# alexj94/future_urban_scene_generation

Hardware: AMD Instinct MI355X
Metric: synthesised vehicle crops/sec @256x256 (higher is better)
Workload: dtype f32 tensors; conv contraction as 3 fp16 MFMA products of scaled (hi, lo) operand splits, f32 accumulate (error vs fp64 <= 1.3x the exact-f32 MFMA kernel's: observed 0.96-1.27x over 12 operand scales x 5 layers; range-guarded; exact-f32 leg in precision_legs)

## Files before the change

### future_urban_scene_generation_amd/_lib.py

```python
from __future__ import annotations

import ctypes as C
import os

_HERE = os.path.dirname(os.path.abspath(__file__))
LIB_PATH = os.environ.get("FUSG_LIB", os.path.join(_HERE, "libfusg.so"))


class FusgUnavailable(RuntimeError):
    pass


class FusgError(RuntimeError):
    pass


class Tensor(C.Structure):
    _fields_ = [("data", C.c_void_p),
                ("n", C.c_int64), ("c", C.c_int64), ("h", C.c_int64), ("w", C.c_int64),
                ("sn", C.c_int64), ("sc", C.c_int64), ("sh", C.c_int64), ("sw", C.c_int64),
                ("dtype", C.c_int32), ("_pad", C.c_int32)]


class ConvDesc(C.Structure):
# ... 72 lines not shown
    "fusg_set_route_batch": (C.c_int, [C.c_int32]),
    "fusg_route_batch": (C.c_int32, []),
    "fusg_conv2d_route_order": (C.c_int, [C.POINTER(ConvDesc), C.POINTER(C.c_int32 * 4)]),
    "fusg_hg_bottleneck": (C.c_int, [C.POINTER(BneckDesc), C.c_void_p]),
    "fusg_vunet_respair": (C.c_int, [C.POINTER(RespairDesc), C.c_void_p]),
    "fusg_hg_head": (C.c_int, [C.POINTER(HgHeadDesc), C.c_void_p]),
    "fusg_conv2d_entry_nin": (C.c_int, [C.POINTER(ConvDesc), C.POINTER(ConvDesc), C.c_void_p]),
    "fusg_conv2d_entry_nin_route": (C.c_int, [C.POINTER(ConvDesc), C.POINTER(ConvDesc)]),
    "fusg_chan_stats": (C.c_int, [_TP, C.c_void_p, C.c_int32, C.c_void_p]),
    "fusg_in_finalize": (C.c_int, [_TP, C.c_void_p, C.c_int32, C.c_float, C.c_void_p, C.c_void_p, C.c_void_p]),
    "fusg_ln_finalize": (C.c_int, [_TP, C.c_void_p, C.c_int32, C.c_float, C.c_void_p, C.c_void_p, C.c_void_p,
                                   C.c_void_p, C.c_void_p]),
    "fusg_in_finalize_slots": (C.c_int, [C.c_void_p, C.c_int32, C.c_int32, C.c_int32, C.c_float, C.c_void_p, C.c_void_p, C.c_void_p]),
    "fusg_ln_finalize_slots": (C.c_int, [C.c_void_p, C.c_int32, C.c_int32, C.c_int32, C.c_float, C.c_void_p, C.c_void_p,
                                         C.c_void_p, C.c_void_p, C.c_void_p]),
    "fusg_affine_act": (C.c_int, [_TP, C.c_void_p, C.c_void_p, C.c_int64, C.c_int32, _TP, _TP, C.c_void_p]),
    "fusg_maxpool2": (C.c_int, [_TP, _TP, C.c_void_p]),
    "fusg_upsample2_add": (C.c_int, [_TP, _TP, _TP, C.c_void_p]),
    "fusg_copy4d": (C.c_int, [_TP, _TP, C.c_int32, C.c_void_p]),
    "fusg_add4d": (C.c_int, [_TP, _TP, _TP, C.c_void_p]),
    "fusg_space_to_depth2": (C.c_int, [_TP, _TP, C.c_void_p]),
    "fusg_depth_to_space2": (C.c_int, [_TP, _TP, C.c_void_p]),
    "fusg_ec_inputs": (C.c_int, [_TP, _TP, _TP, _TP, C.c_int32, C.c_void_p]),
    "fusg_hshift_sum": (C.c_int, [_TP, C.c_void_p, C.c_int32, C.c_int32, C.c_int32, C.c_int32, _TP, C.c_void_p]),
    "fusg_argmax_hw": (C.c_int, [_TP, C.c_void_p, C.c_void_p]),
    "fusg_to_image_u8": (C.c_int, [_TP, _TP, C.c_void_p]),
    "fusg_merge_u8": (C.c_int, [_TP, _TP, _TP, _TP, C.c_void_p]),
    "fusg_warp_perspective_u8": (C.c_int, [_TP, C.c_void_p, _TP, C.c_void_p]),
    "fusg_warp_perspective_indexed_u8": (C.c_int, [_TP, C.c_void_p, C.c_void_p, C.c_int32, _TP, C.c_void_p]),
    "fusg_warp_perspective_frames_u8": (C.c_int, [_TP, C.c_void_p, C.c_void_p, C.c_int32, C.c_int32, _TP, C.c_void_p]),
# ... 146 lines not shown
```

### future_urban_scene_generation_amd/csrc/conv_igemm.hip

```cpp
#include <stdlib.h>
#include <mutex>
#include "conv_kernel_tapunit.h"
#include "conv_kernel_small.h"
#include "conv_kernel_tapunit_f32.h"

namespace fusg {

__global__ __launch_bounds__(256) void conv_splitk_reduce(const ConvK p, int nphase) {
    const int n4 = p.Cout_pad >> 2;
    const long total = (long)nphase * p.M * n4;
    const long idx = (long)blockIdx.x * 256 + threadIdx.x;
    if (idx >= total) return;
    const int c4 = (int)(idx % n4);
    const long pm = idx / n4;
    const int m = (int)(pm % p.M);
    const int phase = (int)(pm / p.M);
    f32x4 s = {0.f, 0.f, 0.f, 0.f};
    const float* base = p.ws + ((long)phase * p.ksplit * p.M + m) * p.Cout_pad + c4 * 4;
    const long slab = (long)p.M * p.Cout_pad;
    int k = 0;
    for (; k + 8 <= p.ksplit; k += 8) {
        f32x4 v[8];
#pragma unroll
        for (int j = 0; j < 8; ++j) v[j] = *(const f32x4*)(base + (long)(k + j) * slab);
// ... 330 lines not shown

    plan_impl(d, &r->sc);
    FUSG_CHECK(d->tile >= 1 && d->tile <= 5, "conv2d: tile %d", d->tile);
    FUSG_CHECK(d->cout_pad % kTiles[d->tile].bn == 0, "conv2d: cout_pad %d not a multiple of tile N %d", d->cout_pad, kTiles[d->tile].bn);
    {
        auto vec_ok = [](const fusg_tensor& t) {
            return t.sc == 1 && (((uintptr_t)t.data) & 15) == 0 && t.sw % 4 == 0 && t.sh % 4 == 0 && t.sn % 4 == 0;
        };
        bool v = d->cout % 4 == 0 && d->dst_c_off % 4 == 0 && vec_ok(o) && !env_switches().no_vec_epi;
        if (d->store_mode == FUSG_STORE_D2S) v = v && (d->cout / 4) % 4 == 0;
        if (d->res0.data) v = v && vec_ok(d->res0);
        if (d->res1.data) v = v && vec_ok(d->res1);
        r->vec_epi = v ? 1 : 0;
    }
    if (d->stats_out) {
        if (!(r->vec_epi && d->act == FUSG_ACT_NONE && !d->res0.data && !d->res1.data && d->store_mode == FUSG_STORE_NORMAL &&
              nphase == 1 && d->ksplit <= 1 && ((long)d->qh * d->qw) % 32 == 0)) {
            set_error("conv2d: fused statistics need act NONE, no residual, NORMAL store, nphase 1, ksplit 1, qh*qw%%32==0 "
                      "and a channel-contiguous aligned dst with cout%%4==0");
            return FUSG_ERR_UNSUPPORTED;
        }
        const int slots = (int)(((long)d->qh * d->qw) / 32);
        if (d->stats_slots > 0 && d->stats_slots < slots) { set_error("conv2d: stats_slots %d < %d slots of this launch", d->stats_slots, slots); return FUSG_ERR_INVALID; }
    }

    const int ntaps = d->kh * d->kw;
    if (r->sc.ksplit > 0) { r->family = FUSG_CONV_SMALL; return FUSG_OK; }
    if ((d->precision == FUSG_PREC_F16X3 || d->precision == FUSG_PREC_F32) && getenv("FUSG_NO_POINTWISE") == nullptr && nphase == 1 && d->kh == 1 && d->kw == 1 && d->stride == 1 && d->upsample == 0 && !has1 &&
        d->c0k >= 4 && d->c0k <= 8 && d->ksplit <= 1 && d->store_mode == FUSG_STORE_NORMAL && r->vec_epi && !d->stats_out &&
        d->cout % 4 == 0 && d->pre_op <= FUSG_PRE_ELU && (d->q_oy | d->q_ox) == 0 && !d->tile_list && d->wpack && d->pad_h == 0 &&
        d->pad_w == 0 && 256 % (d->cout_pad >> 2) == 0 && !env_switches().no_halo && !env_switches().no_pointwise) {
        r->family = FUSG_CONV_POINTWISE;
        return FUSG_OK;
// ... 336 lines not shown
```

### future_urban_scene_generation_amd/csrc/norm.hip

```cpp
#include "common.h"

namespace fusg {

typedef float f32x4 __attribute__((ext_vector_type(4)));

__global__ __launch_bounds__(256) void chan_stats_kernel(const float* __restrict__ x, float* __restrict__ partial,
                                                         int HW, int C, int Cs, int nchunk) {
    __shared__ f32x4 red[2][256];
    const int C4 = C >> 2;
    const int cg0 = blockIdx.z * 64;
    const int nq = min(64, C4 - cg0);
    int pl = 256 / nq;
    pl = 1 << (31 - __clz(pl));
    const int t = threadIdx.x;
    const int q = t % nq;
    const int pj = t / nq;
    const int b = blockIdx.y;
    const int chunk = blockIdx.x;
    const int per = (HW + nchunk - 1) / nchunk;
    const int p0 = chunk * per;
    const int p1 = min(HW, p0 + per);
    f32x4 s1 = {0.f, 0.f, 0.f, 0.f}, s2 = {0.f, 0.f, 0.f, 0.f};
    if (pj < pl) {
        const float* xb = x + (long)b * HW * Cs + (cg0 + q) * 4;
// ... 143 lines not shown
        if (t < w) { red[0][t] += red[0][t + w]; red[1][t] += red[1][t + w]; red[2][t] += red[2][t + w]; }
        __syncthreads();
    }
    const double mean = red[0][0] / (double)total;
    double m2 = red[2][0] + 32.0 * (red[1][0] - red[0][0] * mean);
    if (m2 < 0.0) m2 = 0.0;
    const double sd = sqrt(m2 / (32.0 * (double)total - 1.0));
    const double inv = 1.0 / (sd + (double)eps);
    for (int c = t; c < C; c += 1024) {
        const double sc = (double)gamma[c] * inv;
        scale[(long)b * C + c] = (float)sc;
        shift[(long)b * C + c] = (float)((double)beta[c] - mean * sc);
    }
}

}

using namespace fusg;

static int in_finalize_slots_impl(const float* slots, int32_t batch, int32_t nslots, int32_t channels, float eps,
                                      float* scale, float* shift, void* stream) {
    FUSG_CHECK(slots && scale && shift && batch >= 1 && nslots >= 1 && channels >= 1, "in_finalize_slots: bad arguments");
    hipLaunchKernelGGL(in_finalize_slots_kernel, dim3((channels + 15) / 16, batch), dim3(256), 0, (hipStream_t)stream, slots,
                       nslots, channels, eps, scale, shift);
    FUSG_LAUNCH_CHECK("in_finalize_slots");
    return FUSG_OK;
}
extern "C" int fusg_in_finalize_slots(const float* slots, int32_t batch, int32_t nslots, int32_t channels, float eps, float* scale, float* shift, void* stream) { return fusg::plan_dispatch(in_finalize_slots_impl, stream, slots, batch, nslots, channels, eps, scale, shift); }

static int ln_finalize_slots_impl(const float* slots, int32_t batch, int32_t nslots, int32_t channels, float eps,
                                      const float* gamma, const float* beta, float* scale, float* shift, void* stream) {
    FUSG_CHECK(slots && scale && shift && gamma && beta && batch >= 1 && nslots >= 1 && channels >= 1 &&
               (long)nslots * channels * 32 > 1, "ln_finalize_slots: bad arguments");
// ... 44 lines not shown
```

### future_urban_scene_generation_amd/ops.py

```python
from __future__ import annotations

import ctypes as C
from typing import Optional, Tuple

import torch

from . import _lib as L
from .pack import ConvPlan

_DT = {torch.float32: L.F32, torch.uint8: L.U8, torch.int32: L.I32}

import contextlib as _contextlib
import os as _os
from types import SimpleNamespace as _SimpleNamespace
import numpy as _np


def _env_set(name: str) -> bool:
    return name in _os.environ


_PREC = {"f32": L.PREC_F32, "f16x3": L.PREC_F16X3,
         "bf16": L.PREC_BF16,
         "f16": L.PREC_F16,
# ... 411 lines not shown
                ff = plan.frag_f32_dev()
                if ff is not None:
                    d.wfrag_f32 = ff.data_ptr()
                    if RECORDER is not None:
                        RECORDER.keep.append(ff)
    return d, out


def conv(plan: ConvPlan, x0: torch.Tensor, x1: Optional[torch.Tensor] = None, *, out: Optional[torch.Tensor] = None,
         out_c_off: int = 0, res0: Optional[torch.Tensor] = None, res1: Optional[torch.Tensor] = None,
         pre_op: int = L.PRE_NONE, pre: Optional[Tuple[torch.Tensor, torch.Tensor]] = None, pre_bstride: int = 0,
         act: int = L.ACT_NONE, store: int = L.STORE_NORMAL, nchw_out: bool = False, tile: int = L.TILE_AUTO,
         ksplit: int = 0, precision: Optional[str] = None, want_stats: bool = False,
         out_stride: int = 1, out_off: Tuple[int, int] = (0, 0), tiles: Optional[torch.Tensor] = None,
         q_window: Optional[Tuple[int, int, int, int]] = None, q_size: Optional[Tuple[int, int]] = None,
         stats_into: Optional[Tuple[torch.Tensor, int]] = None, tap_sparse: Optional[int] = None):
    d, out = _conv_desc(plan, x0, x1, out=out, out_c_off=out_c_off, res0=res0, res1=res1, pre_op=pre_op, pre=pre,
                        pre_bstride=pre_bstride, act=act, store=store, nchw_out=nchw_out, tile=tile, ksplit=ksplit,
                        precision=precision, want_stats=want_stats, out_stride=out_stride, out_off=out_off, tiles=tiles,
                        q_window=q_window, q_size=q_size, tap_sparse=tap_sparse)
    b, qh, qw = x0.shape[0], d.qh, d.qw
    lib = L.lib()
    nbytes = lib.fusg_conv2d_plan(C.byref(d))
    ws = None
    if nbytes > 0:
        ws = _workspace(x0.device, nbytes)
        d.workspace = ws.data_ptr()
        if _env_set("FUSG_SPLITK_IN_LAUNCH"):
            d.splitk_counters = _splitk_counters(x0.device).data_ptr()
            d.splitk_counters_len = N_COUNTERS
    stats = None
    if want_stats:
        if (d.ksplit <= 1 and plan.nphase == 1 and store == L.STORE_NORMAL and act == L.ACT_NONE and res0 is None
                and res1 is None and (qh * qw) % 32 == 0 and plan.cout % 4 == 0 and out_c_off % 4 == 0 and is_nhwc(out)
                and out.stride(3) % 4 == 0 and not _env_set("FUSG_NO_VEC_EPI") and q_window is None and tiles is None):
            stats = torch.empty((b, qh * qw // 32, plan.cout, 2), device=x0.device, dtype=torch.float32)
            d.stats_out = stats.data_ptr()
    if stats_into is not None:
        buf, first = stats_into
        assert buf.dtype == torch.float32 and buf.is_contiguous() and buf.shape[0] == b and buf.shape[2] == plan.cout
        assert (qh * qw) % 32 == 0 and first + qh * qw // 32 <= buf.shape[1]
        d.stats_out = buf.data_ptr() + first * plan.cout * 2 * 4
        d.stats_slots = int(buf.shape[1])
    L.check(lib.fusg_conv2d(C.byref(d), stream_ptr()), "conv2d")
    return (out, stats) if want_stats else out


def bottleneck_ok(p: dict, x: torch.Tensor, precision: Optional[str] = None) -> bool:
    prec = precision or PRECISION
    if prec not in ("f16x3", "f32") or _env_set("FUSG_NO_BNECK") or (prec == "f32" and (_env_set("FUSG_NO_BNECK_F32") or _env_set("FUSG_NO_F32_HALO"))):
        return False
    c1, c2, c3 = p["c1"], p["c2"], p["c3"]
    if not (c1.cout in (64, 128) and c2.cout == c1.cout and c3.cout == 2 * c1.cout and c1.kh == 1 and c2.kh == 3 and c3.kh == 1
            and c1.c0k == x.shape[1] and x.shape[1] % 32 == 0 and c1.c1k == 0 and c2.pad == 1 and c2.stride == 1):
# ... 224 lines not shown
    key = (h, w, str(device))
    t = _BORDER_TILES.get(key)
    if t is None:
        ny, nx = h // 8, w // 16
        idx = [y * nx + x for y in range(ny) for x in range(nx) if y in (0, ny - 1) or x in (0, nx - 1)]
        t = torch.tensor(idx, dtype=torch.int32, device=device)
        _BORDER_TILES[key] = t
    return t


def up2_phases_ok(x: torch.Tensor, precision: Optional[str] = None) -> bool:
    b, c, h, w = x.shape
    return h >= 2 and w >= 2 and _os.environ.get("FUSG_NO_UP2_PHASES") is None


def conv_up2(exact: ConvPlan, phases, x: torch.Tensor, *, pre_op: int = L.PRE_NONE, pre=None, pre_bstride: int = 0,
             precision: Optional[str] = None, ring: Optional[dict] = None) -> torch.Tensor:
    if phases is None or not up2_phases_ok(x, precision):
        return conv(exact, x, pre_op=pre_op, pre=pre, pre_bstride=pre_bstride, precision=precision)
    b, c, h, w = x.shape
    out = nhwc_empty(b, exact.cout, 2 * h, 2 * w, x.device)
    halo = (((precision or PRECISION) in ("f16x3", "bf16", "f16") or ((precision or PRECISION) == "f32" and not _env_set("FUSG_NO_F32_HALO")))
            and c % 32 == 0 and h % 8 == 0 and w % 16 == 0 and _os.environ.get("FUSG_NO_HALO") is None)
    if isinstance(phases, ConvPlan):
        conv(phases, x, out=out, store=L.STORE_D2S, pre_op=pre_op, pre=pre, pre_bstride=pre_bstride,
             precision=precision, ksplit=1 if halo else 0)
    else:
        for ph, plan in enumerate(phases):
            conv(plan, x, out=out, out_stride=2, out_off=(ph >> 1, ph & 1), pre_op=pre_op, pre=pre,
                 pre_bstride=pre_bstride, precision=precision, ksplit=1 if halo else 0)
    if ring is not None:
        from .pack import up2_ring_launches
        for ry, rx, win, off in up2_ring_launches(h, w):
            if win[2] > 0 and win[3] > 0:
                conv(ring[(ry, rx)], x, out=out, q_window=win, out_stride=2, out_off=off, pre_op=pre_op, pre=pre,
                     pre_bstride=pre_bstride, precision=precision)
        return out
    for win in ((0, 0, 1, 2 * w), (2 * h - 1, 0, 1, 2 * w), (0, 0, 2 * h, 1), (0, 2 * w - 1, 2 * h, 1)):
        conv(exact, x, out=out, q_window=win, pre_op=pre_op, pre=pre, pre_bstride=pre_bstride, precision=precision)
    return out


def conv_transpose_phases(phases, x: torch.Tensor, *, pre_op: int = L.PRE_NONE, pre=None, pre_bstride: int = 0,
                          act: int = L.ACT_NONE, want_stats: bool = False, precision: Optional[str] = None):
    b, c, h, w = x.shape
    cout = phases[0].cout
    out = nhwc_empty(b, cout, 2 * h, 2 * w, x.device)
    n = h * w // 32
    fuse = (want_stats and act == L.ACT_NONE and (h * w) % 32 == 0 and cout % 4 == 0
            and _os.environ.get("FUSG_NO_VEC_EPI") is None)
    stats = torch.empty((b, 4 * n, cout, 2), device=x.device, dtype=torch.float32) if fuse else None
    for ph, plan in enumerate(phases):
        conv(plan, x, out=out, out_stride=2, out_off=(ph >> 1, ph & 1), q_size=(h, w), pre_op=pre_op, pre=pre,
             pre_bstride=pre_bstride, act=act, precision=precision, ksplit=1,
             stats_into=(stats, ph * n) if fuse else None)
# ... 1059 lines not shown
```

### future_urban_scene_generation_amd/pack.py

```python
from __future__ import annotations

from dataclasses import dataclass, field
from typing import List,  Optional, Sequence, Tuple

import numpy as np
import torch

BK = 32


def _ru(x: int, m: int) -> int:
    return (x + m - 1) // m * m


@dataclass
class ConvPlan:
    wpack: torch.Tensor
    bias: torch.Tensor
    ktab: torch.Tensor
    cout: int
    cout_pad: int
    k_pad: int
    c_split: Tuple[int, ...]
    c0k: int
# ... 268 lines not shown
    out = []
    for ry, Y0, py in (("f", 0, 0), ("l", h - 1, 1)):
        out += [(ry, "e", (Y0, 1, 1, w - 1), (py, 0)), (ry, "o", (Y0, 0, 1, w - 1), (py, 1)),
                (ry, "f", (Y0, 0, 1, 1), (py, 0)), (ry, "l", (Y0, w - 1, 1, 1), (py, 1))]
    for rx, X0, px in (("f", 0, 0), ("l", w - 1, 1)):
        out += [("e", rx, (1, X0, h - 1, 1), (0, px)), ("o", rx, (0, X0, h - 1, 1), (1, px))]
    return out


def pack_conv_up2_ring(weight: torch.Tensor, bias: Optional[torch.Tensor]) -> dict:
    from . import _lib as L
    kinds = sorted({(ry, rx) for ry, rx, _, _ in up2_ring_launches(4, 4)})
    return {k: pack_conv(up2_border_weights(weight, *k), bias, stride=1, pad=1, pad_mode=L.PAD_REPLICATE) for k in kinds}


def pack_conv_up2_d2s(weight: torch.Tensor, bias: Optional[torch.Tensor]) -> ConvPlan:
    from . import _lib as L
    ws = torch.cat(up2_phase_weights(weight), dim=0)
    bs = None if bias is None else bias.detach().to("cpu", torch.float32).repeat(4)
    return pack_conv(ws, bs, stride=1, pad=1, pad_mode=L.PAD_REPLICATE)


def pack_conv_up2_phases(weight: torch.Tensor, bias: Optional[torch.Tensor]) -> List[ConvPlan]:
    from . import _lib as L
    return [pack_conv(wp, bias, stride=1, pad=1, pad_mode=L.PAD_REPLICATE) for wp in up2_phase_weights(weight)]


TAP_SPARSE_NEAREST, TAP_SPARSE_TRANSPOSE = 1, 2
TAP_SPARSE_AXIS = {TAP_SPARSE_NEAREST: ((0, 1), (1, 2)), TAP_SPARSE_TRANSPOSE: ((1,), (1, 2))}
UP2K3_ROWMAP = ((0, 1, 1), (1, 1, 2))
# ... 139 lines not shown
```

### future_urban_scene_generation_amd/warp_learn/models.py

```python
from __future__ import annotations

from typing import List, Optional

import torch
import torch.nn as nn

from .. import _lib as L
from .. import ops, pack
from ..nn_base import ConvP, FusedNet, dev_vec, entry_point


class LayerNorm(nn.Module):

    def __init__(self, num_features: int, eps: float = 1e-5, affine: bool = True):
        super().__init__()
        self.num_features, self.eps, self.affine = num_features, eps, affine
        if affine:
            self.gamma = nn.Parameter(torch.Tensor(num_features).uniform_())
            self.beta = nn.Parameter(torch.zeros(num_features))


class Conv2dBlock(nn.Module):

    def __init__(self, input_dim, output_dim, kernel_size, stride, padding=0, norm="none", activation="relu",
# ... 68 lines not shown
            return pack.pack_conv_rowsplit(blk.conv.weight, blk.conv.bias, pad=blk.padding, pad_mode=L.PAD_REFLECT).to(device)
        return self._pack_block(blk, device)

    def _pack_res(self, rbs: ResBlocks, device) -> List[tuple]:
        return [(self._pack_block(rb.model[0], device), self._pack_block(rb.model[1], device)) for rb in rbs.model]

    def _build_plans(self, device) -> dict:
        enc, dec = self.enc_content.model, self.dec.model
        nd = self.num_downs
        stem = enc[0]
        P = {"stem": pack.pack_conv(stem.conv.weight, stem.conv.bias, stride=1, pad=stem.padding, pad_mode=L.PAD_REFLECT,
                                    cin_pad=4).to(device),
             "down": [self._pack_block(enc[1 + i], device) for i in range(nd)],
             "enc_res": self._pack_res(enc[1 + nd], device),
             "dec_res": self._pack_res(dec[0], device),
             "up": [], "up_phases": [], "up_ring": [], "ln": [],
             "head": self._pack_head(dec[1 + 2 * nd], device)}
        for i in range(nd):
            blk = dec[2 + 2 * i]
            P["up"].append(self._pack_block(blk, device, upsample=1))
            ok = blk.kernel_size == 5 and blk.padding == 2 and blk.stride == 1 and blk.pad_type == "reflect"
            ok = ok and blk.conv.weight.shape[0] % 4 == 0
            P["up_phases"].append(pack.pack_conv_up2_d2s(blk.conv.weight, blk.conv.bias).to(device) if ok else None)
            P["up_ring"].append({k: v.to(device) for k, v in pack.pack_conv_up2_ring(blk.conv.weight, blk.conv.bias).items()}
                                if ok and ops._env_set("FUSG_UP2_RING9") else None)
            P["ln"].append((dev_vec(blk.norm.gamma, device), dev_vec(blk.norm.beta, device), blk.norm.eps))
        return P

    @staticmethod
    def _resblocks(plans, y: torch.Tensor) -> torch.Tensor:
        for pa, pb in plans:
            a, sa = ops.conv_in(pa, y)
            b, sb = ops.conv_in(pb, a, pre_op=L.PRE_AFFINE_RELU, pre=sa, pre_bstride=a.shape[1])
            y = ops.affine_act(b, sb[0], sb[1], L.ACT_NONE, res=y)
        return y

    def _encode(self, P, x: torch.Tensor) -> torch.Tensor:
        c, st = ops.conv_in(P["stem"], ops.as_nhwc(x, cpad=P["stem"].c0k))
        for p in P["down"]:
            c, st = ops.conv_in(p, c, pre_op=L.PRE_AFFINE_RELU, pre=st, pre_bstride=c.shape[1])
        y = ops.affine_act(c, st[0], st[1], L.ACT_RELU)
        return self._resblocks(P["enc_res"], y)

    def _decode(self, P, y: torch.Tensor) -> torch.Tensor:
        y = self._resblocks(P["dec_res"], y)
        pre_op, pre, bs = L.PRE_NONE, None, 0
        for p, ph, rg, (gamma, beta, eps) in zip(P["up"], P["up_phases"], P["up_ring"], P["ln"]):
            if ph is not None and ops.up2_phases_ok(y):
                y = ops.conv_up2(p, ph, y, pre_op=pre_op, pre=pre, pre_bstride=bs, ring=rg)
                pre = ops.layernorm_stats(y, gamma, beta, eps)
            else:
                y, pre = ops.conv_ln(p, y, gamma, beta, eps, pre_op=pre_op, pre=pre, pre_bstride=bs)
            pre_op, bs = L.PRE_AFFINE_RELU, y.shape[1]
        if P["head"].rowsplit is not None:
            return ops.conv_rowsplit(P["head"], y, pre_op=pre_op, pre=pre, pre_bstride=bs, act=L.ACT_TANH)
        return ops.conv(P["head"], y, pre_op=pre_op, pre=pre, pre_bstride=bs, act=L.ACT_TANH, nchw_out=True)

    @entry_point
    def decode(self, content: torch.Tensor) -> torch.Tensor:
        P = self._ensure(content)
        return self._decode(P, ops.as_nhwc(content))

    @entry_point
    def forward(self, image: torch.Tensor) -> torch.Tensor:
        P = self._ensure(image)
# ... 101 lines not shown
```

### include/fusg.h

```cpp
#ifndef FUSG_H
#define FUSG_H

#include <stdint.h>

#ifdef __cplusplus
extern "C" {
#endif

#define FUSG_VERSION 118

typedef enum fusg_status {
    FUSG_OK = 0,
    FUSG_ERR_INVALID = -1,
    FUSG_ERR_LAUNCH = -2,
    FUSG_ERR_UNSUPPORTED = -3
} fusg_status;

typedef enum fusg_dtype { FUSG_F32 = 0, FUSG_U8 = 1, FUSG_I32 = 2 } fusg_dtype;

typedef struct fusg_tensor {
    void*   data;
    int64_t n, c, h, w;
    int64_t sn, sc, sh, sw;
    int32_t dtype;
// ... 152 lines not shown
int fusg_pack_conv_weights(const fusg_pack_spec* spec, const float* weight, const float* bias, float* wpack, int32_t* ktab,
                           float* bias_pad, uint16_t* wpack_h, float* wscale, uint16_t* wfrag);


int fusg_chan_stats(const fusg_tensor* x, float* partial, int32_t nchunk, void* stream);
int fusg_in_finalize(const fusg_tensor* x, const float* partial, int32_t nchunk, float eps,
                     float* scale, float* shift, void* stream);
int fusg_ln_finalize(const fusg_tensor* x, const float* partial, int32_t nchunk, float eps,
                     const float* gamma, const float* beta, float* scale, float* shift, void* stream);

int fusg_in_finalize_slots(const float* slots, int32_t batch, int32_t nslots, int32_t channels, float eps,
                           float* scale, float* shift, void* stream);
int fusg_ln_finalize_slots(const float* slots, int32_t batch, int32_t nslots, int32_t channels, float eps,
                           const float* gamma, const float* beta, float* scale, float* shift, void* stream);


int fusg_affine_act(const fusg_tensor* x, const float* scale, const float* shift, int64_t bstride,
                    int32_t act, const fusg_tensor* res, const fusg_tensor* dst, void* stream);
int fusg_maxpool2(const fusg_tensor* x, const fusg_tensor* dst, void* stream);
int fusg_upsample2_add(const fusg_tensor* low, const fusg_tensor* up1, const fusg_tensor* dst, void* stream);
int fusg_copy4d(const fusg_tensor* src, const fusg_tensor* dst, int32_t dst_c_fill, void* stream);
int fusg_add4d(const fusg_tensor* a, const fusg_tensor* b, const fusg_tensor* dst, void* stream);
int fusg_space_to_depth2(const fusg_tensor* x, const fusg_tensor* dst, void* stream);
int fusg_depth_to_space2(const fusg_tensor* x, const fusg_tensor* dst, void* stream);
int fusg_ec_inputs(const fusg_tensor* images, const fusg_tensor* edges, const fusg_tensor* masks,
                   const fusg_tensor* dst, int32_t mode, void* stream);
int fusg_hshift_sum(const fusg_tensor* t, const float* bias, int32_t kw, int32_t pad, int32_t pad_mode,
                    int32_t act, const fusg_tensor* dst, void* stream);
int fusg_argmax_hw(const fusg_tensor* x, int32_t* idx, void* stream);
int fusg_to_image_u8(const fusg_tensor* x, const fusg_tensor* dst, void* stream);
// ... 229 lines not shown
```

Measured before the change: 1562.

## Fix up2 conv borders with an edge-correction kernel and fuse LayerNorm stats

Upsample-by-2 decoder convs now run the D2S phase conv over the whole image. A new MFMA kernel then adds a border correction along the four image edges, instead of running separate border-window convs. The conv also emits fused LayerNorm statistics in D2S store mode. The edge kernel records per-segment deltas of sum and sum of squares, and a new finalize kernel folds these into the statistics, which removes the separate layernorm_stats pass over the output. The cost is extra complexity and a double-precision correction formula whose numerics have to match.

After: 1594 (median of 6 runs). 2.1% higher.

```diff
diff --git a/future_urban_scene_generation_amd/_lib.py b/future_urban_scene_generation_amd/_lib.py
--- a/future_urban_scene_generation_amd/_lib.py
+++ b/future_urban_scene_generation_amd/_lib.py
@@ -110,6 +110,10 @@
     "fusg_in_finalize_slots": (C.c_int, [C.c_void_p, C.c_int32, C.c_int32, C.c_int32, C.c_float, C.c_void_p, C.c_void_p, C.c_void_p]),
     "fusg_ln_finalize_slots": (C.c_int, [C.c_void_p, C.c_int32, C.c_int32, C.c_int32, C.c_float, C.c_void_p, C.c_void_p,
                                          C.c_void_p, C.c_void_p, C.c_void_p]),
+    "fusg_up2_edge_entries": (C.c_int, [C.c_int32, C.c_int32]),
+    "fusg_up2_edge_fix": (C.c_int, [_TP, C.c_int32, C.c_void_p, C.c_void_p, C.c_int64, C.c_void_p, _TP, C.c_void_p, C.c_int32, C.c_void_p]),
+    "fusg_ln_finalize_slots_delta": (C.c_int, [C.c_void_p, C.c_int32, C.c_int32, C.c_int32, C.c_int32, C.c_float, C.c_void_p, C.c_void_p,
+                                               C.c_void_p, C.c_int32, C.c_void_p, C.c_void_p, C.c_void_p]),
     "fusg_affine_act": (C.c_int, [_TP, C.c_void_p, C.c_void_p, C.c_int64, C.c_int32, _TP, _TP, C.c_void_p]),
     "fusg_maxpool2": (C.c_int, [_TP, _TP, C.c_void_p]),
     "fusg_upsample2_add": (C.c_int, [_TP, _TP, _TP, C.c_void_p]),
diff --git a/future_urban_scene_generation_amd/csrc/conv_igemm.hip b/future_urban_scene_generation_amd/csrc/conv_igemm.hip
--- a/future_urban_scene_generation_amd/csrc/conv_igemm.hip
+++ b/future_urban_scene_generation_amd/csrc/conv_igemm.hip
@@ -368,9 +368,10 @@
         r->vec_epi = v ? 1 : 0;
     }
     if (d->stats_out) {
-        if (!(r->vec_epi && d->act == FUSG_ACT_NONE && !d->res0.data && !d->res1.data && d->store_mode == FUSG_STORE_NORMAL &&
+        if (!(r->vec_epi && d->act == FUSG_ACT_NONE && !d->res0.data && !d->res1.data &&
+              (d->store_mode == FUSG_STORE_NORMAL || d->store_mode == FUSG_STORE_D2S) &&
               nphase == 1 && d->ksplit <= 1 && ((long)d->qh * d->qw) % 32 == 0)) {
-            set_error("conv2d: fused statistics need act NONE, no residual, NORMAL store, nphase 1, ksplit 1, qh*qw%%32==0 "
+            set_error("conv2d: fused statistics need act NONE, no residual, NORMAL or D2S store, nphase 1, ksplit 1, qh*qw%%32==0 "
                       "and a channel-contiguous aligned dst with cout%%4==0");
             return FUSG_ERR_UNSUPPORTED;
         }
diff --git a/future_urban_scene_generation_amd/csrc/norm.hip b/future_urban_scene_generation_amd/csrc/norm.hip
--- a/future_urban_scene_generation_amd/csrc/norm.hip
+++ b/future_urban_scene_generation_amd/csrc/norm.hip
@@ -181,9 +181,60 @@
     }
 }
 
+__global__ __launch_bounds__(1024) void ln_finalize_slots_delta_kernel(const float* __restrict__ slots, int nslots, int cols, int C,
+                                                                       float eps, const float* __restrict__ gamma,
+                                                                       const float* __restrict__ beta, const double* __restrict__ delta,
+                                                                       int nent, float* __restrict__ scale, float* __restrict__ shift) {
+    __shared__ double red[3][1024];
+    const int b = blockIdx.x, t = threadIdx.x;
+    const long total = (long)nslots * cols;
+    const float2* s = (const float2*)slots + (long)b * total;
+    double sm = 0.0, sq = 0.0, s2 = 0.0;
+#pragma unroll 4
+    for (long k = t; k < total; k += 1024) {
+        const float2 v = s[k];
+        sm += (double)v.x;
+        sq += (double)v.x * (double)v.x;
+        s2 += (double)v.y;
+    }
+    red[0][t] = sm; red[1][t] = sq; red[2][t] = s2;
+    __syncthreads();
+    for (int w = 512; w > 0; w >>= 1) {
+        if (t < w) { red[0][t] += red[0][t + w]; red[1][t] += red[1][t + w]; red[2][t] += red[2][t + w]; }
+        __syncthreads();
+    }
+    double d1 = 0.0, d2 = 0.0;
+    for (int k = 0; k < nent; ++k) { d1 += delta[((long)b * nent + k) * 2]; d2 += delta[((long)b * nent + k) * 2 + 1]; }
+    const double n = 32.0 * (double)total;
+    const double S1 = 32.0 * red[0][0] + d1;
+    const double mean = S1 / n;
+    const double m0 = red[0][0] / (double)total;
+    double m2 = red[2][0] + 32.0 * (red[1][0] - red[0][0] * m0) + (d2 - 2.0 * m0 * d1) - n * (mean - m0) * (mean - m0);
+    if (m2 < 0.0) m2 = 0.0;
+    const double sd = sqrt(m2 / (n - 1.0));
+    const double inv = 1.0 / (sd + (double)eps);
+    for (int c = t; c < C; c += 1024) {
+        const double sc = (double)gamma[c] * inv;
+        scale[(long)b * C + c] = (float)sc;
+        shift[(long)b * C + c] = (float)((double)beta[c] - mean * sc);
+    }
+}
+
 }
 
 using namespace fusg;
+
+static int ln_finalize_slots_delta_impl(const float* slots, int32_t batch, int32_t nslots, int32_t columns, int32_t channels, float eps,
+                                        const float* gamma, const float* beta, const double* delta, int32_t n_entries,
+                                        float* scale, float* shift, void* stream) {
+    FUSG_CHECK(slots && scale && shift && gamma && beta && delta && batch >= 1 && nslots >= 1 && columns >= 1 && channels >= 1 &&
+               n_entries >= 1 && (long)nslots * columns * 32 > 1, "ln_finalize_slots_delta: bad arguments");
+    hipLaunchKernelGGL(ln_finalize_slots_delta_kernel, dim3((unsigned)batch), dim3(1024), 0, (hipStream_t)stream, slots, nslots,
+                       columns, channels, eps, gamma, beta, delta, n_entries, scale, shift);
+    FUSG_LAUNCH_CHECK("ln_finalize_slots_delta");
+    return FUSG_OK;
+}
+extern "C" int fusg_ln_finalize_slots_delta(const float* slots, int32_t batch, int32_t nslots, int32_t columns, int32_t channels, float eps, const float* gamma, const float* beta, const double* delta, int32_t n_entries, float* scale, float* shift, void* stream) { return fusg::plan_dispatch(ln_finalize_slots_delta_impl, stream, slots, batch, nslots, columns, channels, eps, gamma, beta, delta, n_entries, scale, shift); }
 
 static int in_finalize_slots_impl(const float* slots, int32_t batch, int32_t nslots, int32_t channels, float eps,
                                       float* scale, float* shift, void* stream) {
diff --git a/future_urban_scene_generation_amd/csrc/up2_edge.h b/future_urban_scene_generation_amd/csrc/up2_edge.h
--- /dev/null
+++ b/future_urban_scene_generation_amd/csrc/up2_edge.h
@@ -0,0 +1,26 @@
+#pragma once
+#include "common.h"
+
+namespace fusg {
+
+constexpr int UP2E_CH = 32;
+constexpr int UP2E_PITCH = UP2E_CH + 4;
+
+struct Up2EdgeK {
+    const float* src;
+    long ssn, ssh, ssw;
+    int h, w, Cin, Cout;
+    int pre_relu_affine;
+    const float* pre_scale;
+    const float* pre_shift;
+    long pre_bstride;
+    const float* wedge;
+    float* dst;
+    long dsn, dsh, dsw;
+    double* delta;
+    int n_entries, entry0;
+    int axis;
+    int nseg;
+};
+
+}
diff --git a/future_urban_scene_generation_amd/csrc/up2_edge.hip b/future_urban_scene_generation_amd/csrc/up2_edge.hip
--- /dev/null
+++ b/future_urban_scene_generation_amd/csrc/up2_edge.hip
@@ -0,0 +1,234 @@
+#include "up2_edge.h"
+
+namespace fusg {
+
+typedef float f32x4 __attribute__((ext_vector_type(4)));
+
+template <int RT, int CTW>
+__global__ __launch_bounds__(256) void up2_edge_kernel(const Up2EdgeK p) {
+    constexpr int SEG = RT * 16, NE = SEG + 4, ITEMS = NE * (UP2E_CH / 4), NIT = (ITEMS + 255) / 256;
+    __shared__ __attribute__((aligned(16))) float lds[2][NE * UP2E_PITCH];
+    __shared__ double red[2][4];
+    const int t = threadIdx.x, lane = t & 63, wave = t >> 6;
+    const int seg = blockIdx.x, side = blockIdx.y, b = blockIdx.z;
+    const int l = p.axis == 0 ? p.w : p.h, L = 2 * l;
+    const int la = p.axis == 0 ? p.h : p.w;
+    const int a1 = side == 0 ? 1 : la - 2, a0 = side == 0 ? 0 : la - 1;
+    const long s_al = p.axis == 0 ? p.ssw : p.ssh, s_ac = p.axis == 0 ? p.ssh : p.ssw;
+    const float* s1 = p.src + (long)b * p.ssn + (long)a1 * s_ac;
+    const float* s0 = p.src + (long)b * p.ssn + (long)a0 * s_ac;
+    const int p0 = seg * SEG;
+    const int q4 = (t & 7) * 4;
+
+    long off1[NIT], off0[NIT];
+    bool live[NIT];
+#pragma unroll
+    for (int k = 0; k < NIT; ++k) {
+        const int el = (t + 256 * k) >> 3;
+        const int P = p0 - 2 + el;
+        int j1 = 0, j0 = 0;
+        bool ok = el < NE && P <= L + 1;
+        if (P == -2) { j1 = 1; j0 = 0; ok = ok && p.axis == 0; }
+        else if (P == L + 1) { j1 = l - 2; j0 = l - 1; ok = ok && p.axis == 0; }
+        else if (ok) { const int c = P < 0 ? 0 : (P > L - 1 ? L - 1 : P); j1 = j0 = c >> 1; }
+        live[k] = ok;
+        off1[k] = (long)j1 * s_al + q4;
+        off0[k] = (long)j0 * s_al + q4;
+    }
+    const float* sc_p = p.pre_relu_affine ? p.pre_scale + (long)b * p.pre_bstride + q4 : nullptr;
+    const float* sh_p = p.pre_relu_affine ? p.pre_shift + (long)b * p.pre_bstride + q4 : nullptr;
+
+    f32x4 v1[NIT], v0[NIT], sc = {1.f, 1.f, 1.f, 1.f}, sh = {0.f, 0.f, 0.f, 0.f};
+    auto fetch = [&](int c) {
+        const int c0 = c * UP2E_CH;
+        if (p.pre_relu_affine) { sc = *(const f32x4*)(sc_p + c0); sh = *(const f32x4*)(sh_p + c0); }
+#pragma unroll
+        for (int k = 0; k < NIT; ++k) {
+            if (live[k]) { v1[k] = *(const f32x4*)(s1 + off1[k] + c0); v0[k] = *(const f32x4*)(s0 + off0[k] + c0); }
+        }
+    };
+    auto stage = [&](float* buf) {
+#pragma unroll
+        for (int k = 0; k < NIT; ++k) {
+            const int el = (t + 256 * k) >> 3;
+            if (el >= NE) continue;
+            f32x4 d = {0.f, 0.f, 0.f, 0.f};
+            if (live[k]) {
+                f32x4 a = v1[k], c = v0[k];
+                if (p.pre_relu_affine) {
+#pragma unroll
+                    for (int e = 0; e < 4; ++e) { a[e] = fmaxf(fmaf(a[e], sc[e], sh[e]), 0.f); c[e] = fmaxf(fmaf(c[e], sc[e], sh[e]), 0.f); }
+                }
+                d = a - c;
+            }
+            *(f32x4*)(buf + el * UP2E_PITCH + q4) = d;
+        }
+    };
+
+    const int nct = p.Cout >> 4, nc16 = p.Cin >> 4, nchunk = p.Cin / UP2E_CH;
+    const int gside = 2 * p.axis + side;
+    const bool active = wave * CTW < nct;
+    f32x4 acc[RT][CTW];
+#pragma unroll
+    for (int i = 0; i < RT; ++i)
+#pragma unroll
+        for (int j = 0; j < CTW; ++j) acc[i][j] = f32x4{0.f, 0.f, 0.f, 0.f};
+
+    constexpr bool AHEAD = CTW <= 2;
+    f32x4 bw[5][2][CTW], bwn[5][2][CTW];
+    auto fetch_w = [&](int c, f32x4 (&dstw)[5][2][CTW]) {
+#pragma unroll
+        for (int tap = 0; tap < 5; ++tap)
+#pragma unroll
+            for (int hh = 0; hh < 2; ++hh)
+#pragma unroll
+                for (int j = 0; j < CTW; ++j) {
+                    const int ct = wave * CTW + j;
+                    dstw[tap][hh][j] = f32x4{0.f, 0.f, 0.f, 0.f};
+                    if (ct < nct)
+                        dstw[tap][hh][j] = *(const f32x4*)(p.wedge + ((((long)(gside * 5 + tap) * nc16 + (2 * c + hh)) * nct + ct) * 64 + lane) * 4);
+                }
+    };
+
+    if (active) fetch_w(0, bw);
+    fetch(0);
+    stage(lds[0]);
+    __syncthreads();
+    for (int c = 0; c < nchunk; ++c) {
+        if (c + 1 < nchunk) {
+            fetch(c + 1);
+            if (AHEAD && active) fetch_w(c + 1, bwn);
+        }
+        if (active) {
+            const float* buf = lds[c & 1];
+#pragma unroll
+            for (int tap = 0; tap < 5; ++tap)
+#pragma unroll
+                for (int hh = 0; hh < 2; ++hh) {
+                    f32x4 a[RT];
+#pragma unroll
+                    for (int i = 0; i < RT; ++i)
+                        a[i] = *(const f32x4*)(buf + (i * 16 + (lane & 15) + tap) * UP2E_PITCH + hh * 16 + (lane >> 4) * 4);
+#pragma unroll
+                    for (int e = 0; e < 4; ++e)
+#pragma unroll
+                        for (int i = 0; i < RT; ++i)
+#pragma unroll
+                            for (int j = 0; j < CTW; ++j)
+                                acc[i][j] = __builtin_amdgcn_mfma_f32_16x16x4f32(a[i][e], bw[tap][hh][j][e], acc[i][j], 0, 0, 0);
+                }
+        }
+        if (c + 1 < nchunk) {
+            stage(lds[(c + 1) & 1]);
+            if (active) {
+                if (AHEAD) {
+#pragma unroll
+                    for (int tap = 0; tap < 5; ++tap)
+#pragma unroll
+                        for (int hh = 0; hh < 2; ++hh)
+#pragma unroll
+                            for (int j = 0; j < CTW; ++j) bw[tap][hh][j] = bwn[tap][hh][j];
+                } else {
+                    fetch_w(c + 1, bw);
+                }
+            }
+        }
+        __syncthreads();
+    }
+
+    const long d_al = p.axis == 0 ? p.dsw : p.dsh;
+    float* dline = p.dst + (long)b * p.dsn + (p.axis == 0 ? (side ? 2L * p.h - 1 : 0L) * p.dsh : (side ? 2L * p.w - 1 : 0L) * p.dsw);
+    double sd = 0.0, sq = 0.0;
+    if (active) {
+#pragma unroll
+        for (int i = 0; i < RT; ++i)
+#pragma unroll
+            for (int j = 0; j < CTW; ++j) {
+                const int ct = wave * CTW + j;
+                if (ct >= nct) continue;
+#pragma unroll
+                for (int r = 0; r < 4; ++r) {
+                    const int pp = p0 + i * 16 + (lane >> 4) * 4 + r;
+                    if (pp >= L) continue;
+                    float* o = dline + (long)pp * d_al + ct * 16 + (lane & 15);
+                    const float old = *o;
+                    const float nw = old + acc[i][j][r];
+                    *o = nw;
+                    const double de = (double)nw - (double)old;
+                    sd += de;
+                    sq += de * (2.0 * (double)old + de);
+                }
+            }
+    }
+    if (p.delta != nullptr) {
+#pragma unroll
+        for (int off = 32; off > 0; off >>= 1) { sd += __shfl_xor(sd, off, 64); sq += __shfl_xor(sq, off, 64); }
+        if (lane == 0) { red[0][wave] = sd; red[1][wave] = sq; }
+        __syncthreads();
+        if (t == 0) {
+            double* e = p.delta + ((long)b * p.n_entries + p.entry0 + side * p.nseg + seg) * 2;
+            e[0] = ((red[0][0] + red[0][1]) + red[0][2]) + red[0][3];
+            e[1] = ((red[1][0] + red[1][1]) + red[1][2]) + red[1][3];
+        }
+    }
+}
+
+static inline int up2_edge_rt(long L) { return L >= 256 ? 4 : 2; }
+static inline int up2_edge_nseg(long L) { const int seg = 16 * up2_edge_rt(L); return (int)((L + seg - 1) / seg); }
+
+template <int RT>
+static void up2_edge_launch_rt(const Up2EdgeK& k, dim3 grid, hipStream_t s) {
+    if (k.Cout <= 64) hipLaunchKernelGGL((up2_edge_kernel<RT, 1>), grid, dim3(256), 0, s, k);
+    else if (k.Cout <= 128) hipLaunchKernelGGL((up2_edge_kernel<RT, 2>), grid, dim3(256), 0, s, k);
+    else hipLaunchKernelGGL((up2_edge_kernel<RT, 4>), grid, dim3(256), 0, s, k);
+}
+
+}
+
+using namespace fusg;
+
+static int up2_edge_impl(const fusg_tensor* src, int32_t pre_op, const float* pre_scale, const float* pre_shift, int64_t pre_bstride,
+                         const float* wedge, const fusg_tensor* dst, double* delta, int32_t n_entries, void* stream) {
+    FUSG_CHECK(src && dst && is_nhwc(*src) && is_nhwc(*dst) && wedge && (((uintptr_t)wedge) & 15) == 0, "up2_edge_fix: src / dst must be NHWC-physical, weights 16-byte aligned");
+    FUSG_CHECK(src->h >= 2 && src->w >= 2 && src->h < (1 << 14) && src->w < (1 << 14) && src->n >= 1 && src->n <= 65535,
+               "up2_edge_fix: low-res image %ld x %ld, batch %ld", (long)src->h, (long)src->w, (long)src->n);
+    FUSG_CHECK(dst->n == src->n && dst->h == 2 * src->h && dst->w == 2 * src->w, "up2_edge_fix: dst is not the 2x image of src");
+    FUSG_CHECK(src->c >= 32 && src->c % 32 == 0 && dst->c >= 16 && dst->c % 16 == 0 && dst->c <= 256,
+               "up2_edge_fix: Cin %ld (multiple of 32) / Cout %ld (multiple of 16, <= 256)", (long)src->c, (long)dst->c);
+    FUSG_CHECK(pre_op == FUSG_PRE_NONE || pre_op == FUSG_PRE_AFFINE_RELU, "up2_edge_fix: pre_op %d", pre_op);
+    if (pre_op == FUSG_PRE_AFFINE_RELU)
+        FUSG_CHECK(pre_scale && pre_shift && ((((uintptr_t)pre_scale) | ((uintptr_t)pre_shift)) & 15) == 0 && pre_bstride % 4 == 0 && pre_bstride >= 0,
+                   "up2_edge_fix: affine pre-op needs 16-byte aligned scale / shift");
+    const int nsw = up2_edge_nseg(2 * src->w), nsh = up2_edge_nseg(2 * src->h);
+    FUSG_CHECK(!delta || (n_entries == 2 * nsw + 2 * nsh && (((uintptr_t)delta) & 7) == 0), "up2_edge_fix: delta buffer needs %d entries per image, got %d",
+               2 * nsw + 2 * nsh, n_entries);
+    Up2EdgeK k{};
+    k.src = (const float*)src->data; k.ssn = src->sn; k.ssh = src->sh; k.ssw = src->sw;
+    k.h = (int)src->h; k.w = (int)src->w; k.Cin = (int)src->c; k.Cout = (int)dst->c;
+    k.pre_relu_affine = pre_op == FUSG_PRE_AFFINE_RELU;
+    k.pre_scale = pre_scale; k.pre_shift = pre_shift; k.pre_bstride = pre_bstride;
+    k.wedge = wedge;
+    k.dst = (float*)dst->data; k.dsn = dst->sn; k.dsh = dst->sh; k.dsw = dst->sw;
+    k.delta = delta; k.n_entries = n_entries;
+    for (int axis = 0; axis < 2; ++axis) {
+        const long L = 2 * (axis == 0 ? src->w : src->h);
+        k.axis = axis;
+        k.nseg = axis == 0 ? nsw : nsh;
+        k.entry0 = axis == 0 ? 0 : 2 * nsw;
+        const dim3 grid((unsigned)k.nseg, 2, (unsigned)src->n);
+        if (up2_edge_rt(L) == 4) up2_edge_launch_rt<4>(k, grid, (hipStream_t)stream);
+        else up2_edge_launch_rt<2>(k, grid, (hipStream_t)stream);
+        FUSG_LAUNCH_CHECK("up2_edge_fix");
+    }
+    return FUSG_OK;
+}
+
+extern "C" int fusg_up2_edge_entries(int32_t h, int32_t w) {
+    if (h < 2 || w < 2) return 0;
+    return 2 * up2_edge_nseg(2L * w) + 2 * up2_edge_nseg(2L * h);
+}
+
+extern "C" int fusg_up2_edge_fix(const fusg_tensor* src, int32_t pre_op, const float* pre_scale, const float* pre_shift, int64_t pre_bstride,
+                                 const float* wedge, const fusg_tensor* dst, double* delta, int32_t n_entries, void* stream) {
+    return fusg::plan_dispatch(up2_edge_impl, stream, src, pre_op, pre_scale, pre_shift, pre_bstride, wedge, dst, delta, n_entries);
+}
diff --git a/future_urban_scene_generation_amd/ops.py b/future_urban_scene_generation_amd/ops.py
--- a/future_urban_scene_generation_amd/ops.py
+++ b/future_urban_scene_generation_amd/ops.py
@@ -449,7 +449,7 @@
          ksplit: int = 0, precision: Optional[str] = None, want_stats: bool = False,
          out_stride: int = 1, out_off: Tuple[int, int] = (0, 0), tiles: Optional[torch.Tensor] = None,
          q_window: Optional[Tuple[int, int, int, int]] = None, q_size: Optional[Tuple[int, int]] = None,
-         stats_into: Optional[Tuple[torch.Tensor, int]] = None, tap_sparse: Optional[int] = None):
+         stats_into: Optional[Tuple[torch.Tensor, int]] = None, tap_sparse: Optional[int] = None, stats_d2s: bool = False):
     d, out = _conv_desc(plan, x0, x1, out=out, out_c_off=out_c_off, res0=res0, res1=res1, pre_op=pre_op, pre=pre,
                         pre_bstride=pre_bstride, act=act, store=store, nchw_out=nchw_out, tile=tile, ksplit=ksplit,
                         precision=precision, want_stats=want_stats, out_stride=out_stride, out_off=out_off, tiles=tiles,
@@ -466,13 +466,15 @@
             d.splitk_counters_len = N_COUNTERS
     stats = None
     if want_stats:
-        if (d.ksplit <= 1 and plan.nphase == 1 and store == L.STORE_NORMAL and act == L.ACT_NONE and res0 is None
+        if (d.ksplit <= 1 and plan.nphase == 1 and (store == L.STORE_NORMAL or (stats_d2s and store == L.STORE_D2S and plan.cout % 16 == 0))
+                and act == L.ACT_NONE and res0 is None
                 and res1 is None and (qh * qw) % 32 == 0 and plan.cout % 4 == 0 and out_c_off % 4 == 0 and is_nhwc(out)
                 and out.stride(3) % 4 == 0 and not _env_set("FUSG_NO_VEC_EPI") and q_window is None and tiles is None):
             stats = torch.empty((b, qh * qw // 32, plan.cout, 2), device=x0.device, dtype=torch.float32)
             d.stats_out = stats.data_ptr()
     if stats_into is not None:
         buf, first = stats_into
+        assert store == L.STORE_NORMAL
         assert buf.dtype == torch.float32 and buf.is_contiguous() and buf.shape[0] == b and buf.shape[2] == plan.cout
         assert (qh * qw) % 32 == 0 and first + qh * qw // 32 <= buf.shape[1]
         d.stats_out = buf.data_ptr() + first * plan.cout * 2 * 4
@@ -727,15 +729,57 @@
     return h >= 2 and w >= 2 and _os.environ.get("FUSG_NO_UP2_PHASES") is None
 
 
+def up2_edge_ok(edge, phases, x: torch.Tensor, pre_op: int, ring) -> bool:
+    return (edge is not None and isinstance(phases, ConvPlan) and ring is None and not _env_set("FUSG_NO_UP2_EDGE")
+            and pre_op in (L.PRE_NONE, L.PRE_AFFINE_RELU) and x.shape[1] == edge.cin and is_nhwc(x))
+
+
+def up2_edge_fix(edge, x: torch.Tensor, out: torch.Tensor, *, pre_op: int = L.PRE_NONE, pre=None, pre_bstride: int = 0,
+                 want_delta: bool = False) -> Optional[torch.Tensor]:
+    b, c, h, w = x.shape
+    lib = L.lib()
+    delta, n = None, 0
+    if want_delta:
+        n = int(lib.fusg_up2_edge_entries(h, w))
+        delta = torch.empty((b, n, 2), device=x.device, dtype=torch.float64)
+    if RECORDER is not None:
+        RECORDER.keep.append(edge.w)
+        if pre is not None:
+            RECORDER.keep.append(pre)
+    L.check(lib.fusg_up2_edge_fix(C.byref(desc(x)), int(pre_op), pre[0].data_ptr() if pre is not None else None,
+                                  pre[1].data_ptr() if pre is not None else None, int(pre_bstride), edge.w.data_ptr(),
+                                  C.byref(desc(out)), delta.data_ptr() if delta is not None else None, n, stream_ptr()), "up2_edge_fix")
+    return delta
+
+
 def conv_up2(exact: ConvPlan, phases, x: torch.Tensor, *, pre_op: int = L.PRE_NONE, pre=None, pre_bstride: int = 0,
-             precision: Optional[str] = None, ring: Optional[dict] = None) -> torch.Tensor:
+             precision: Optional[str] = None, ring: Optional[dict] = None, edge=None, ln=None):
+    def with_ln(o, ss=None):
+        if ln is None:
+            return o
+        return o, (ss if ss is not None else layernorm_stats(o, ln[0], ln[1], ln[2]))
+
     if phases is None or not up2_phases_ok(x, precision):
-        return conv(exact, x, pre_op=pre_op, pre=pre, pre_bstride=pre_bstride, precision=precision)
+        return with_ln(conv(exact, x, pre_op=pre_op, pre=pre, pre_bstride=pre_bstride, precision=precision))
     b, c, h, w = x.shape
     out = nhwc_empty(b, exact.cout, 2 * h, 2 * w, x.device)
     halo = (((precision or PRECISION) in ("f16x3", "bf16", "f16") or ((precision or PRECISION) == "f32" and not _env_set("FUSG_NO_F32_HALO")))
             and c % 32 == 0 and h % 8 == 0 and w % 16 == 0 and _os.environ.get("FUSG_NO_HALO") is None)
-    if isinstance(phases, ConvPlan):
+    if up2_edge_ok(edge, phases, x, pre_op, ring):
+        r = conv(phases, x, out=out, store=L.STORE_D2S, pre_op=pre_op, pre=pre, pre_bstride=pre_bstride,
+                 precision=precision, ksplit=1 if halo else 0, want_stats=ln is not None, stats_d2s=True)
+        stats = r[1] if ln is not None else None
+        if ln is None or stats is not None:
+            delta = up2_edge_fix(edge, x, out, pre_op=pre_op, pre=pre, pre_bstride=pre_bstride, want_delta=stats is not None)
+            if ln is None:
+                return out
+            nslots, cols = stats.shape[1], stats.shape[2]
+            ss = torch.empty((2, b, exact.cout), device=x.device, dtype=torch.float32)
+            L.check(L.lib().fusg_ln_finalize_slots_delta(stats.data_ptr(), b, nslots, cols, exact.cout, float(ln[2]), ln[0].data_ptr(),
+                                                         ln[1].data_ptr(), delta.data_ptr(), delta.shape[1], ss[0].data_ptr(),
+                                                         ss[1].data_ptr(), stream_ptr()), "ln_finalize_slots_delta")
+            return out, (ss[0], ss[1])
+    elif isinstance(phases, ConvPlan):
         conv(phases, x, out=out, store=L.STORE_D2S, pre_op=pre_op, pre=pre, pre_bstride=pre_bstride,
              precision=precision, ksplit=1 if halo else 0)
     else:
@@ -748,10 +792,10 @@
             if win[2] > 0 and win[3] > 0:
                 conv(ring[(ry, rx)], x, out=out, q_window=win, out_stride=2, out_off=off, pre_op=pre_op, pre=pre,
                      pre_bstride=pre_bstride, precision=precision)
-        return out
+        return with_ln(out)
     for win in ((0, 0, 1, 2 * w), (2 * h - 1, 0, 1, 2 * w), (0, 0, 2 * h, 1), (0, 2 * w - 1, 2 * h, 1)):
         conv(exact, x, out=out, q_window=win, pre_op=pre_op, pre=pre, pre_bstride=pre_bstride, precision=precision)
-    return out
+    return with_ln(out)
 
 
 def conv_transpose_phases(phases, x: torch.Tensor, *, pre_op: int = L.PRE_NONE, pre=None, pre_bstride: int = 0,
diff --git a/future_urban_scene_generation_amd/pack.py b/future_urban_scene_generation_amd/pack.py
--- a/future_urban_scene_generation_amd/pack.py
+++ b/future_urban_scene_generation_amd/pack.py
@@ -306,6 +306,74 @@
     return {k: pack_conv(up2_border_weights(weight, *k), bias, stride=1, pad=1, pad_mode=L.PAD_REPLICATE) for k in kinds}
 
 
+UP2_EDGE_SIDES = ("top", "bottom", "left", "right")
+
+
+def up2_edge_taps(weight: torch.Tensor) -> torch.Tensor:
+    w = weight.detach().to("cpu")
+    assert w.shape[2] == 5 and w.shape[3] == 5, w.shape
+    return torch.stack([w[:, :, 0, :], w[:, :, 4, :], w[:, :, :, 0], w[:, :, :, 4]]).permute(0, 3, 1, 2).contiguous()
+
+
+@dataclass
+class Up2Edge:
+    w: torch.Tensor
+    cin: int
+    cout: int
+
+    def to(self, device) -> "Up2Edge":
+        self.w = self.w.to(device)
+        return self
+
+    def taps(self) -> torch.Tensor:
+        v = self.w.reshape(4, 5, self.cin // 16, self.cout // 16, 4, 16, 4)
+        return v.permute(0, 1, 3, 5, 2, 4, 6).reshape(4, 5, self.cout, self.cin)
+
+
+def pack_conv_up2_edge(weight: torch.Tensor) -> Optional[Up2Edge]:
+    cout, cin = weight.shape[:2]
+    if cin % 32 or cout % 16 or cout > 256 or cin < 32:
+        return None
+    t = up2_edge_taps(weight.detach().to("cpu", torch.float32))
+    v = t.reshape(4, 5, cout // 16, 16, cin // 16, 4, 4)
+    return Up2Edge(w=v.permute(0, 1, 4, 2, 5, 3, 6).reshape(4, 5, cin // 16, cout // 16, 64, 4).contiguous(), cin=cin, cout=cout)
+
+
+def up2_edge_frame(fx: torch.Tensor):
+    b, c, h, w = fx.shape
+
+    def line(a1, a0, L, corner0, corner1):
+        j = (torch.arange(-2, L + 2).clamp(0, L - 1) // 2)
+        e = (a1 - a0)[:, :, j].clone()
+        e[:, :, 0], e[:, :, L + 3] = corner0, corner1
+        return e
+
+    z = torch.zeros_like(fx[:, :, 0, 0])
+    return [line(fx[:, :, 1, :], fx[:, :, 0, :], 2 * w, fx[:, :, 1, 1] - fx[:, :, 0, 0], fx[:, :, 1, w - 2] - fx[:, :, 0, w - 1]),
+            line(fx[:, :, h - 2, :], fx[:, :, h - 1, :], 2 * w, fx[:, :, h - 2, 1] - fx[:, :, h - 1, 0],
+                 fx[:, :, h - 2, w - 2] - fx[:, :, h - 1, w - 1]),
+            line(fx[:, :, :, 1], fx[:, :, :, 0], 2 * h, z, z),
+            line(fx[:, :, :, w - 2], fx[:, :, :, w - 1], 2 * h, z, z)]
+
+
+def up2_edge_delta(taps: torch.Tensor, fx: torch.Tensor) -> torch.Tensor:
+    b, c, h, w = fx.shape
+    out = torch.zeros(b, taps.shape[2], 2 * h, 2 * w, dtype=fx.dtype)
+    tp = taps.to(fx.dtype)
+    for side, e in enumerate(up2_edge_frame(fx)):
+        L = e.shape[2] - 4
+        d = sum(torch.einsum("oc,bcp->bop", tp[side, t], e[:, :, t:t + L]) for t in range(5))
+        if side == 0:
+            out[:, :, 0, :] += d
+        elif side == 1:
+            out[:, :, 2 * h - 1, :] += d
+        elif side == 2:
+            out[:, :, :, 0] += d
+        else:
+            out[:, :, :, 2 * w - 1] += d
+    return out
+
+
 def pack_conv_up2_d2s(weight: torch.Tensor, bias: Optional[torch.Tensor]) -> ConvPlan:
     from . import _lib as L
     ws = torch.cat(up2_phase_weights(weight), dim=0)
diff --git a/future_urban_scene_generation_amd/warp_learn/models.py b/future_urban_scene_generation_amd/warp_learn/models.py
--- a/future_urban_scene_generation_amd/warp_learn/models.py
+++ b/future_urban_scene_generation_amd/warp_learn/models.py
@@ -106,7 +106,7 @@
              "down": [self._pack_block(enc[1 + i], device) for i in range(nd)],
              "enc_res": self._pack_res(enc[1 + nd], device),
              "dec_res": self._pack_res(dec[0], device),
-             "up": [], "up_phases": [], "up_ring": [], "ln": [],
+             "up": [], "up_phases": [], "up_ring": [], "up_edge": [], "ln": [],
              "head": self._pack_head(dec[1 + 2 * nd], device)}
         for i in range(nd):
             blk = dec[2 + 2 * i]
@@ -116,6 +116,8 @@
             P["up_phases"].append(pack.pack_conv_up2_d2s(blk.conv.weight, blk.conv.bias).to(device) if ok else None)
             P["up_ring"].append({k: v.to(device) for k, v in pack.pack_conv_up2_ring(blk.conv.weight, blk.conv.bias).items()}
                                 if ok and ops._env_set("FUSG_UP2_RING9") else None)
+            ed = pack.pack_conv_up2_edge(blk.conv.weight) if ok else None
+            P["up_edge"].append(ed.to(device) if ed is not None else None)
             P["ln"].append((dev_vec(blk.norm.gamma, device), dev_vec(blk.norm.beta, device), blk.norm.eps))
         return P
 
@@ -137,10 +139,9 @@
     def _decode(self, P, y: torch.Tensor) -> torch.Tensor:
         y = self._resblocks(P["dec_res"], y)
         pre_op, pre, bs = L.PRE_NONE, None, 0
-        for p, ph, rg, (gamma, beta, eps) in zip(P["up"], P["up_phases"], P["up_ring"], P["ln"]):
+        for p, ph, rg, ed, (gamma, beta, eps) in zip(P["up"], P["up_phases"], P["up_ring"], P["up_edge"], P["ln"]):
             if ph is not None and ops.up2_phases_ok(y):
-                y = ops.conv_up2(p, ph, y, pre_op=pre_op, pre=pre, pre_bstride=bs, ring=rg)
-                pre = ops.layernorm_stats(y, gamma, beta, eps)
+                y, pre = ops.conv_up2(p, ph, y, pre_op=pre_op, pre=pre, pre_bstride=bs, ring=rg, edge=ed, ln=(gamma, beta, eps))
             else:
                 y, pre = ops.conv_ln(p, y, gamma, beta, eps, pre_op=pre_op, pre=pre, pre_bstride=bs)
             pre_op, bs = L.PRE_AFFINE_RELU, y.shape[1]
diff --git a/include/fusg.h b/include/fusg.h
--- a/include/fusg.h
+++ b/include/fusg.h
@@ -190,6 +190,13 @@
 int fusg_ln_finalize_slots(const float* slots, int32_t batch, int32_t nslots, int32_t channels, float eps,
                            const float* gamma, const float* beta, float* scale, float* shift, void* stream);
 
+int fusg_up2_edge_entries(int32_t h, int32_t w);
+int fusg_up2_edge_fix(const fusg_tensor* src, int32_t pre_op, const float* pre_scale, const float* pre_shift, int64_t pre_bstride,
+                      const float* wedge, const fusg_tensor* dst, double* delta, int32_t n_entries, void* stream);
+int fusg_ln_finalize_slots_delta(const float* slots, int32_t batch, int32_t nslots, int32_t columns, int32_t channels, float eps,
+                                 const float* gamma, const float* beta, const double* delta, int32_t n_entries,
+                                 float* scale, float* shift, void* stream);
+
 
 int fusg_affine_act(const fusg_tensor* x, const float* scale, const float* shift, int64_t bstride,
                     int32_t act, const fusg_tensor* res, const fusg_tensor* dst, void* stream);
```
